# fateshelled/sycl_points

Measured on AMD Instinct MI355X. Metric: gicp_correspondences_per_sec, higher is better.
Workload: dtype f32

## Files before the change

sycl_points_amd/_lib.py:

```python
import ctypes as C
import os
import subprocess

_HERE = os.path.dirname(os.path.abspath(__file__))
LIB_PATH = os.environ.get("SP_AMD_LIB") or os.path.join(_HERE, "lib", "libsycl_points_amd.so")
CSRC = os.path.join(_HERE, "csrc")

SP_OK, SP_ERR_INVALID_ARGUMENT, SP_ERR_RUNTIME, SP_ERR_HIP = 0, 1, 2, 3
COMM_ID_BYTES = 128


class SpError(RuntimeError):

    def __init__(self, code, msg):
        super().__init__(f"[sycl_points_amd] error {code}: {msg}")
        self.code = code


class Linearized(C.Structure):
    _fields_ = [("H", C.c_float * 36), ("b", C.c_float * 6), ("error", C.c_float), ("inlier", C.c_uint32),
                ("inlier_lo", C.c_float), ("inlier_hi", C.c_float), ("pad", C.c_float * 2)]


class FactorParams(C.Structure):
# ... 344 lines not shown
    "sp_vhm_downsampling": (_i, [_vp, _vp, _f, _vp, _vp, _vp, _vp, _vp, _sz, C.POINTER(_sz), _vp]),
    "sp_vhm_overlap_ratio": (_i, [_vp, _vp, _sz, _vp, C.POINTER(_f), _vp]),
    "sp_vhm_remove_old_data": (_i, [_vp, _vp]),
    "sp_ogm_create": (_i, [_f, _vp, C.POINTER(_vp)]),
    "sp_ogm_destroy": (None, [_vp]),
    "sp_ogm_set": (_i, [_vp, _i, _f]),
    "sp_ogm_set_log_odds_limits": (_i, [_vp, _f, _f]),
    "sp_ogm_get": (_f, [_vp, _i]),
    "sp_ogm_info": (_sz, [_vp, _i]),
    "sp_ogm_clear": (_i, [_vp, _vp]),
    "sp_ogm_add_point_cloud": (_i, [_vp, _vp, _vp, _vp, _vp, _sz, _vp, _vp]),
    "sp_ogm_extract_occupied_points": (_i, [_vp, _vp, _f, _vp, _vp, _vp, _vp, _vp, _sz, C.POINTER(_sz), _vp]),
    "sp_ogm_extract_visible_points": (_i, [_vp, _vp, _f, _f, _f, _vp, _vp, _vp, _vp, _vp, _sz, C.POINTER(_sz), _vp]),
    "sp_ogm_overlap_ratio": (_i, [_vp, _vp, _sz, _vp, C.POINTER(_f), _vp]),
    "sp_ogm_voxel_probability": (_i, [_vp, _vp, C.POINTER(_f), _vp]),
    "sp_ogm_export": (_i, [_vp, _vp, _vp, _vp, _vp, _vp, _vp, _vp, _vp, _vp, _sz, C.POINTER(_sz), _vp]),
    "sp_pc2_resolve_fields_host": (_i, [C.POINTER(C.c_char_p), C.POINTER(C.c_uint32), C.POINTER(C.c_uint8), _sz, C.c_uint32, _i, _i, _i,
                                        C.POINTER(Pc2Layout)]),
    "sp_pc2_unpack_workspace_bytes": (_sz, [_sz]),
    "sp_pc2_unpack": (_i, [_vp, _sz, _sz, C.POINTER(Pc2Layout), _vp, _vp, _vp, _vp, _vp, _vp, _vp]),
    "sp_pc2_pack_point_step": (C.c_uint32, [_i, _i, _i]),
    "sp_pc2_pack": (_i, [_vp, _vp, _vp, _vp, _sz, C.c_double, _vp, _vp]),
    "sp_enhanced_reflectivity_workspace_bytes": (_sz, [_sz]),
    "sp_enhanced_reflectivity": (_i, [_vp, _vp, _sz, _vp, C.c_uint32, C.c_int32, _i, C.c_int32, _vp, _f, _f, _vp, _vp]),
}


INTERNAL_SIGNATURES = {
    "sp_internal_source_option": (_i, [_vp, _i, _i]),
    "sp_internal_grid_option": (_i, [_vp, _i, _i]),
    "sp_internal_bvh_option": (_i, [_vp, _i, _i]),
    "sp_internal_grid_small_build": (_i, [_i]),
    "sp_internal_align_searched_log": (_vp, [_vp, _vp]),
    "sp_internal_radix_sort_workspace_bytes": (_sz, [_sz]),
    "sp_internal_radix_sort_u32": (_i, [_vp, _vp, _vp, _vp, _sz, C.c_uint, _vp, _sz, _vp, _vp]),
    "sp_internal_radix_sort_u32_ex": (_i, [_vp, _vp, _vp, _vp, _sz, C.c_uint, C.c_uint, _i, _vp, _sz, _vp, _vp]),
    "sp_internal_radix_first_pass": (None, [_sz, C.c_uint, _vp]),
    "sp_internal_radix_sort_u64": (_i, [_vp, _vp, _vp, _vp, _sz, C.c_uint, _vp, _sz, _vp, _vp]),
    "sp_internal_exclusive_scan_workspace_bytes": (_sz, [_sz]),
    "sp_internal_exclusive_scan_u32": (_i, [_vp, _vp, _sz, _vp, _vp, _sz, _vp]),
    "sp_internal_atan2f_host": (None, [_vp, _vp, _sz, _vp]),
    "sp_internal_fps": (_i, [_i, _vp, _sz, _sz, C.c_uint32, _vp, _vp, _vp, _vp, _sz, _vp]),
    "sp_internal_eigen3": (_i, [_vp, _sz, _vp, _vp, _vp]),
    "sp_internal_inverse3": (_i, [_vp, _sz, _vp, _vp]),
}
VOXEL_BOX_SHARDS, VOXEL_BOX_SHARD_STRIDE = 16, 32
COORD = {"LIDAR": 0, "CAMERA": 1}
FPS_FORM = {"auto": 0, "one_workgroup": 1, "per_sample": 2, "persistent": 3}
INTERNAL_OPTION = {"stage_mask": 0, "reuse": 1, "fast_nn": 2, "self_knn_mode": 3, "persistent": 4, "persistent_from": 5,
                   "bvh_self_heap": 6, "bvh_sort_queries": 7, "grid_sort_queries": 8, "opt_wave_query": 9, "opt_fuse_trials": 10}


def build(force=False):
    srcs = [os.path.join(CSRC, f) for f in os.listdir(CSRC) if f.endswith((".hip", ".h"))]
    srcs.append(os.path.join(_HERE, "..", "include", "sycl_points_amd.h"))
    stale = (not os.path.exists(LIB_PATH)) or any(os.path.getmtime(s) > os.path.getmtime(LIB_PATH) for s in srcs)
    if force or stale:
        subprocess.check_call(["make", "-C", CSRC, "-j8", "-s"])
    return LIB_PATH


_lib = None


def lib():
    global _lib
# ... 21 lines not shown
```

sycl_points_amd/csrc/registration.hip:

```cpp
#include <algorithm>
#include <mutex>

#include "registration_device.h"
#include "sp_cov_normal.h"

namespace sp {
namespace {


struct PointTerm {
    float H[6][6];
    float b[6];
    float sq;
    float residual_norm;
    float genz_weight;
};

__device__ __forceinline__ void se3_jacobian(const Rigid& T, float px, float py, float pz, float J[3][6]) {
#pragma unroll
    for (int i = 0; i < 3; ++i) {
        const float r0 = T.R[i][0], r1 = T.R[i][1], r2 = T.R[i][2];
        J[i][0] = chain3(r0, 0.0f, r1, pz, r2, -py);
        J[i][1] = chain3(r0, -pz, r1, 0.0f, r2, px);
        J[i][2] = chain3(r0, py, r1, -px, r2, 0.0f);
// ... 374 lines not shown
    constexpr float kShrink = 0.25f * (1.0f - 1e-3f);
    rho2[o] = fminf(d23[3 * (size_t)i + 1], bound2) * kShrink;
    const int u1 = idx3[3 * (size_t)i + 1];
    float4 r = make_float4(INFINITY, INFINITY, INFINITY, 0.0f);
    if (u1 >= 0) {
        const float4 p = gpts[inv[u1]];
        r.x = p.x; r.y = p.y; r.z = p.z;
    }
    r.w = fminf(d23[3 * (size_t)i + 2], bound2) * kShrink;
    nb[i] = r;
}

__global__ __launch_bounds__(kBlock) void query_cell_kernel(const float4* __restrict__ pts, unsigned n, GridDesc g,
                                                            Mat4Arg T_val, const float* __restrict__ T_dev,
                                                            unsigned* __restrict__ keys, unsigned* __restrict__ vals) {
    const unsigned i = blockIdx.x * kBlock + threadIdx.x;
    if (i >= n) return;
    const Rigid T = load_rigid_colmajor(T_dev ? T_dev : T_val.m);
    const float4 p = pts[i];
    float qx, qy, qz;
    transform_point(T, p.x, p.y, p.z, qx, qy, qz);
    unsigned key = (unsigned)g.nx * g.ny * g.nz;
    if (isfinite(qx) && isfinite(qy) && isfinite(qz)) {
        const int cx = cell_coord(qx, g.ox, g.inv_h, g.nx), cy = cell_coord(qy, g.oy, g.inv_h, g.ny),
                  cz = cell_coord(qz, g.oz, g.inv_h, g.nz);
        key = ((unsigned)cz * g.ny + cy) * g.nx + cx;
    }
    keys[i] = key;
    vals[i] = i;
}
__global__ __launch_bounds__(kBlock) void prepare_source_kernel(const float4* __restrict__ pts,
                                                                const float4* __restrict__ covs,
                                                                unsigned* __restrict__ order, bool identity, unsigned n,
                                                                unsigned stride, float* __restrict__ out_pts,
                                                                float* __restrict__ out_covp) {
    const unsigned i = blockIdx.x * kBlock + threadIdx.x;
    if (i >= n) return;
    const unsigned src = identity ? i : order[i];
    if (identity) order[i] = i;
    const float4 p = pts[src];
    out_pts[i] = p.x; out_pts[stride + i] = p.y; out_pts[2 * (size_t)stride + i] = p.z;
    if (!covs) return;
    const Mat3 P = plane_regularize(load_cov(covs + 4 * (size_t)src));
    out_covp[i] = P.m[0][0];
    out_covp[stride + i] = (P.m[0][1] + P.m[1][0]) * 0.5f;
    out_covp[2 * (size_t)stride + i] = (P.m[0][2] + P.m[2][0]) * 0.5f;
    out_covp[3 * (size_t)stride + i] = P.m[1][1];
    out_covp[4 * (size_t)stride + i] = (P.m[1][2] + P.m[2][1]) * 0.5f;
    out_covp[5 * (size_t)stride + i] = P.m[2][2];
}


template <int LOSS, bool FAST_NN, bool P2D = false>
__global__ __launch_bounds__(kBlock) void gicp_fused_kernel(FusedParams P, float* __restrict__ partials) {
    const Rigid T = load_rigid_colmajor(P.T_dev ? P.T_dev : P.T_val.m);
    float acc[kAcc - 1];
#pragma unroll
    for (int e = 0; e < kAcc - 1; ++e) acc[e] = 0.0f;
    unsigned cnt = 0, searched = 0;
    for (unsigned i = blockIdx.x * kBlock + threadIdx.x; i < P.n; i += gridDim.x * kBlock)
        fused_point<LOSS, FAST_NN, P2D, kSeedSearches, kNegCert>(P, T, i, acc, cnt, searched);
    block_reduce_store<kAcc - 1>(acc, cnt, partials + (size_t)blockIdx.x * kPartial, false, searched);
}

template <int LOSS, bool P2D>
__global__ __launch_bounds__(kBlock) void error_prepared_kernel(FusedParams P, Mat4Arg T_lin_val, const float* T_lin_dev,
                                                                float* __restrict__ partials) {
    const Rigid T = load_rigid_colmajor(P.T_dev ? P.T_dev : P.T_val.m);
    const Rigid TL = load_rigid_colmajor(T_lin_dev ? T_lin_dev : T_lin_val.m);
    float acc[1] = {0.0f};
    unsigned cnt = 0;
    for (unsigned i = blockIdx.x * kBlock + threadIdx.x; i < P.n; i += gridDim.x * kBlock)
        error_prepared_point<LOSS, P2D>(P, T, TL, i, acc, cnt);
    block_reduce_store<1>(acc, cnt, partials + (size_t)blockIdx.x * kPartial);
}


struct AlignState {
    float T[16];
    float T_lin[16];
    float delta[8];
    unsigned converged;
// ... 689 lines not shown
    }
    if (certificates) {
        const int rc2 = build_certificates(t, as_stream(stream));
        if (rc2 != SP_OK) { sp_gicp_target_destroy(t); return rc2; }
    }
    const int rc = sp_gicp_target_update(t, tgt_covs, stream);
    if (rc != SP_OK) { sp_gicp_target_destroy(t); return rc; }
    *out = t;
    return SP_OK;
}
}
}

extern "C" int sp_gicp_target_create(const sp_grid* grid, const float* tgt_covs, size_t n, void* stream,
                                     sp_gicp_target** out) {
    return sp::target_create(grid, tgt_covs, n, true, stream, out);
}
extern "C" int sp_gicp_target_create_plain(const sp_grid* grid, const float* tgt_covs, size_t n, void* stream,
                                           sp_gicp_target** out) {
    return sp::target_create(grid, tgt_covs, n, false, stream, out);
}
extern "C" int sp_gicp_target_certify(sp_gicp_target* t, const float* tgt_covs, void* stream) {
    if (!t || !tgt_covs) return SP_ERR_INVALID_ARGUMENT;
    if (t->rho2 != nullptr) return SP_OK;
    t->note(sp::as_stream(stream));
    const int rc = sp::build_certificates(t, sp::as_stream(stream));
    if (rc != SP_OK) return rc;
    return sp_gicp_target_update(t, tgt_covs, stream);
}
extern "C" int sp_gicp_target_has_certificates(const sp_gicp_target* t) { return t && t->rho2 != nullptr ? 1 : 0; }

extern "C" void sp_gicp_source_destroy(sp_gicp_source* s) {
    if (!s) return;
    (void)hipFree(s->pts); (void)hipFree(s->covp); (void)hipFree(s->perm); (void)hipFree(s->ccache); (void)hipFree(s->ccache2); (void)hipFree(s->qcert); (void)hipFree(s->qcert2); (void)hipFree(s->opt_rows);
    (void)hipFree(s->keys_in); (void)hipFree(s->keys_out); (void)hipFree(s->vals_in); (void)hipFree(s->sort_tmp);
    delete s;
}
extern "C" int sp_gicp_source_create(size_t n_max, sp_gicp_source** out) {
    using namespace sp;
    if (!out) return SP_ERR_INVALID_ARGUMENT;
    *out = nullptr;
    if (n_max >= (1ull << 32)) { sp_set_error("[Registration] more than 2^32 source points"); return SP_ERR_INVALID_ARGUMENT; }
    sp_gicp_source* s = new sp_gicp_source();
    s->n_max = n_max;
    const size_t n = n_max ? n_max : 1;
    s->sort_tmp_bytes = radix_sort_u32_workspace_bytes(n);
    hipError_t e = hipMalloc(&s->pts, (n + 64) * sizeof(float4));
    if (e == hipSuccess) e = hipMalloc(&s->covp, (n + 64) * 2 * sizeof(float4));
    if (e == hipSuccess) e = hipMalloc(&s->perm, n * 4);
    if (e == hipSuccess) e = hipMalloc(&s->ccache, n * 3 * sizeof(float4));
    if (e == hipSuccess) e = hipMalloc(&s->ccache2, std::min<size_t>(n, 2048) * 3 * sizeof(float4));
    s->qcert_points = std::min<size_t>(n, 131072);
    if (e == hipSuccess) e = hipMalloc(&s->qcert, s->qcert_points * sizeof(float4));
    if (e == hipSuccess) e = hipMalloc(&s->qcert2, std::min<size_t>(n, 2048) * sizeof(float4));
    if (e == hipSuccess) e = hipMalloc(&s->opt_rows, sp::kOptRowsBytes);
    if (e == hipSuccess) e = hipMemset(s->opt_rows, 0, sp::kOptRowsBytes);
    if (e == hipSuccess) e = hipMalloc(&s->keys_in, n * 4);
    if (e == hipSuccess) e = hipMalloc(&s->keys_out, n * 4);
    if (e == hipSuccess) e = hipMalloc(&s->vals_in, n * 4);
    if (e == hipSuccess) e = hipMalloc(&s->sort_tmp, s->sort_tmp_bytes ? s->sort_tmp_bytes : 16);
    if (e != hipSuccess) {
        sp_set_error(hipGetErrorString(e));
        sp_gicp_source_destroy(s);
        return SP_ERR_HIP;
    }
    *out = s;
    return SP_OK;
}
extern "C" int sp_gicp_source_prepare(sp_gicp_source* s, const sp_gicp_target* target, const float* src_points,
                                      const float* src_covs, size_t n, const float* transT, int transT_on_device,
                                      int sort_by_cell, void* stream) {
    using namespace sp;
    if (!s || !target) return SP_ERR_INVALID_ARGUMENT;
    if (n > s->n_max) {
        sp_set_error("[sp_gicp_source_prepare] more points than the object was created for");
        return SP_ERR_INVALID_ARGUMENT;
    }
    if (!src_covs && n && target->reg_type == SP_REG_GICP) {
        sp_set_error("[Registration::validate_params] Covariance matrices of source and target must be pre-computed "
                     "before performing GICP matching.");
        return SP_ERR_RUNTIME;
    }
    s->n = n;
    s->sorted = sort_by_cell != 0;
    if (n == 0) return SP_OK;
    hipStream_t st = as_stream(stream);
    const float4* pts = reinterpret_cast<const float4*>(src_points);
    const unsigned nb = div_up(n, kBlock);
    if (sort_by_cell == SP_SOURCE_SORT) {
        Mat4Arg tv;
        for (int i = 0; i < 16; ++i) tv.m[i] = (i % 5 == 0) ? 1.0f : 0.0f;
        if (transT && !transT_on_device)
            for (int i = 0; i < 16; ++i) tv.m[i] = transT[i];
        const GridDesc g = grid_desc(target->grid);
        query_cell_kernel<<<nb, kBlock, 0, st>>>(pts, (unsigned)n, g, tv, transT_on_device ? transT : nullptr, s->keys_in,
                                                 s->vals_in);
        unsigned end_bit = 1;
        while ((1ull << end_bit) <= target->grid->ncells && end_bit < 32) ++end_bit;
        const unsigned begin_bit = end_bit > 16 ? end_bit - 16 : 0;
        bool in_b = false;
        if (radix_sort_pairs_u32(s->keys_in, s->keys_out, s->vals_in, s->perm, n, end_bit, s->sort_tmp, s->sort_tmp_bytes, &in_b,
                                 st, begin_bit) != SP_OK) {
            sp_set_error("[Registration] radix sort of the source failed");
            return SP_ERR_HIP;
        }
        if (!in_b) { unsigned* t = s->perm; s->perm = s->vals_in; s->vals_in = t; }
    }
    s->cache_valid = false;
    s->qcert_valid = false;
    s->cache_target = target;
    s->cache_version = target->version;
    prepare_source_kernel<<<nb, kBlock, 0, st>>>(pts, target->reg_type == SP_REG_GICP ? reinterpret_cast<const float4*>(src_covs) : nullptr,
                                                 s->perm, sort_by_cell != SP_SOURCE_SORT, (unsigned)n,
                                                 (unsigned)((n + 63) / 64 * 64), reinterpret_cast<float*>(s->pts),
                                                 reinterpret_cast<float*>(s->covp));
    return launch_status();
}



extern "C" int sp_gicp_iteration_fused(const sp_gicp_target* target, const sp_gicp_source* source, float* transT,
                                       int transT_on_device, const sp_factor_params* params, const sp_gn_params* gn,
                                       int32_t* nn_idx_out, float* nn_d2_out, sp_linearized* out, float* delta_out8,
                                       void* workspace, size_t workspace_bytes, void* stream) {
    using namespace sp;
    hipStream_t st = as_stream(stream);
    if (!target || !source || !params || !out) return SP_ERR_INVALID_ARGUMENT;
    if (const int rc = check_prepared_reg(target, params); rc != SP_OK) return rc;
    if (gn && !transT_on_device) {
        sp_set_error("[sp_gicp_iteration_fused] the fused Gauss-Newton update needs the pose on the device");
        return SP_ERR_INVALID_ARGUMENT;
    }
    const size_t n = source->n;
    if (n == 0) return zero_async(out, sizeof(sp_linearized), st);
    if (const int rc = check_workspace(workspace, workspace_bytes, n); rc != SP_OK) return rc;
    target->note(st);
    const FusedParams P = make_fused_params(target, source, params, transT, transT_on_device, nn_idx_out, nn_d2_out);
    const bool fills_cache = P.ccache != nullptr && (source->opt_stage_mask & 1);
    const unsigned grid = reduce_grid(n);
    float* partials = static_cast<float*>(workspace);
    const int rc = with_variant(params->robust_type, source_fast_nn(source), params->reg_type == SP_REG_POINT_TO_DISTRIBUTION,
                                [&](auto L, auto FAST_NN, auto P2D) {
        if (source->opt_stage_mask & 1)
            gicp_fused_kernel<L, FAST_NN, P2D><<<grid, kBlock, 0, st>>>(P, partials);
        return SP_OK;
    });
    if (rc != SP_OK) return rc;
    if (fills_cache) { source->cache_valid = true; source->qcert_valid = false; }
// ... 327 lines not shown
        for (int k = 0; k < k_tail; ++k) {
            const int rc = sp_gicp_align_step(target, source, transT_device, params, gn, k, 0, nn_idx_out, nn_d2_out, lin_out,
                                              workspace, workspace_bytes, stream);
            if (rc != SP_OK) { persist_release(guard, st); return rc; }
        }
        return launch_persistent(target, source, transT_device, params, gn, k_tail, max_iterations, nn_idx_out, nn_d2_out, lin_out,
                                 delta_out8, iterations_out, workspace, st, guard);
    }
    for (int k = 0; k < max_iterations; ++k) {
        const int rc = sp_gicp_align_step(target, source, transT_device, params, gn, k, 0, nn_idx_out, nn_d2_out, lin_out,
                                          workspace, workspace_bytes, stream);
        if (rc != SP_OK) return rc;
    }
    return sp_gicp_align_finish(source, transT_device, gn, max_iterations - 1, 0, lin_out, delta_out8, iterations_out,
                                workspace, workspace_bytes, stream);
}

extern "C" int sp_gicp_source_set_persistent(sp_gicp_source* s, int enable) {
    if (!s) return SP_ERR_INVALID_ARGUMENT;
    s->opt_persistent = enable ? 1 : 0;
    return SP_OK;
}

extern "C" int sp_gicp_source_set_wave_per_point(sp_gicp_source* s, int mode) {
    if (!s || mode < 0 || mode > 2) return SP_ERR_INVALID_ARGUMENT;
    s->opt_wave_query = mode;
    return SP_OK;
}

extern "C" const uint32_t* sp_internal_align_searched_log(void* workspace, size_t* n_entries_out) {
    if (n_entries_out) *n_entries_out = sp::kSearchedLog;
    return workspace ? sp::align_ws(workspace).searched_log : nullptr;
}
extern "C" int sp_internal_source_option(sp_gicp_source* s, int option, int value) {
    if (!s) return SP_ERR_INVALID_ARGUMENT;
    switch (option) {
        case SP_INTERNAL_FUSED_STAGE_MASK: s->opt_stage_mask = value; return SP_OK;
        case SP_INTERNAL_FUSED_REUSE: s->opt_reuse = value; s->cache_valid = false; return SP_OK;
        case SP_INTERNAL_FUSED_FAST_NN: s->opt_fast_nn = value; return SP_OK;
        case SP_INTERNAL_FUSED_PERSISTENT: s->opt_persistent = value; return SP_OK;
        case SP_INTERNAL_FUSED_PERSISTENT_FROM: s->opt_persistent_from = value < 0 ? 0 : value; return SP_OK;
        case SP_INTERNAL_OPT_WAVE_QUERY: s->opt_wave_query = value; return SP_OK;
        case SP_INTERNAL_OPT_FUSE_TRIALS: s->opt_fuse_trials = value; return SP_OK;
    }
    return SP_ERR_INVALID_ARGUMENT;
}
```

sycl_points_amd/csrc/registration_device.h:

```cpp
#ifndef SP_REGISTRATION_DEVICE_H
#define SP_REGISTRATION_DEVICE_H

#include "grid_device.h"
#include "radix_sort.h"
#include "sp_xchg.h"

#include <type_traits>

void sp_set_error(const char* msg);

#include "sp_internal.h"

namespace sp {
namespace {

constexpr int kAcc = 29;
constexpr int kPartial = 32;
constexpr int kMaxBlocks = 1024;

template <bool SC1>
__device__ __forceinline__ void store_row_word(float* p, float v) {
    if (SC1) __hip_atomic_store(p, v, __ATOMIC_RELAXED, __HIP_MEMORY_SCOPE_AGENT);
    else *p = v;
}
// ... 155 lines not shown
                                               float crit_trans, float* delta_out8, bool fold_inlier, LdltScratch& w) {
    if (fold_inlier) lin->inlier = (uint32_t)lin->inlier_hi * 4096u + (uint32_t)lin->inlier_lo;
    float H[36], nb[6], delta[6];
#pragma unroll
    for (int i = 0; i < 36; ++i) H[i] = lin->H[i];
#pragma unroll
    for (int i = 0; i < 6; ++i) {
        H[i * 6 + i] = lin->H[i * 6 + i] + lambda * 1.0f;
        nb[i] = -lin->b[i];
    }
    const bool ok = ldlt6_solve(H, nb, delta, w);
    const float nr = sqrtf(delta[0] * delta[0] + delta[1] * delta[1] + delta[2] * delta[2]);
    const float nt = sqrtf(delta[3] * delta[3] + delta[4] * delta[4] + delta[5] * delta[5]);
    const bool conv = ok && (nr < crit_rot) && (nt < crit_trans);
    const Rigid cur = load_rigid_colmajor(T);
    const Rigid upd = rigid_mul(cur, se3_exp(delta));
    store_rigid_colmajor(upd, T);
    if (delta_out8) {
        for (int i = 0; i < 6; ++i) delta_out8[i] = delta[i];
        delta_out8[6] = conv ? 1.0f : 0.0f;
        delta_out8[7] = ok ? 1.0f : 0.0f;
    }
}

struct Sym3 {
    float xx, xy, xz, yy, yz, zz;
};

__device__ __forceinline__ Sym3 load_sym(const float4* __restrict__ p) {
    const float4 a = p[0], b = p[1];
    return Sym3{a.x, a.y, a.z, a.w, b.x, b.y};
}

struct FusedParams {
    const float* src;
    const float* scovp;
    unsigned sstride;
    const float4* tpts;
    const unsigned* tstart;
    const float4* tcovp;
    const float4* tnb;
    GridDesc g;
    unsigned n;
    float max_d2, scale;
    Mat4Arg T_val;
    const float* T_dev;
    const unsigned* perm;
    float4* ccache;
    int cache_valid;
    int32_t* nn_idx;
    float* nn_d2;
};

template <int LOSS, bool P2D = false, bool ERR_ONLY = false, int NACC = kAcc - 1>
__device__ __forceinline__ void fused_math(const FusedParams& P, const Rigid& T, const float4 s, float qx, float qy,
                                           float qz, const Nearest& nn, const Sym3& Cs, const Sym3& Ct,
                                           float (&acc)[NACC], unsigned& cnt) {
    const float r0 = nn.x - qx, r1 = nn.y - qy, r2 = nn.z - qz;
    const float (&R)[3][3] = T.R;
    float W[3][3];
#pragma unroll
    for (int j = 0; j < 3; ++j) {
        W[0][j] = chain3(Ct.xx, R[0][j], Ct.xy, R[1][j], Ct.xz, R[2][j]);
        W[1][j] = chain3(Ct.xy, R[0][j], Ct.yy, R[1][j], Ct.yz, R[2][j]);
        W[2][j] = chain3(Ct.xz, R[0][j], Ct.yz, R[1][j], Ct.zz, R[2][j]);
    }
    const float g00 = chain3(R[0][0], W[0][0], R[1][0], W[1][0], R[2][0], W[2][0]);
    const float g01 = chain3(R[0][0], W[0][1], R[1][0], W[1][1], R[2][0], W[2][1]);
    const float g02 = chain3(R[0][0], W[0][2], R[1][0], W[1][2], R[2][0], W[2][2]);
    const float g11 = chain3(R[0][1], W[0][1], R[1][1], W[1][1], R[2][1], W[2][1]);
    const float g12 = chain3(R[0][1], W[0][2], R[1][1], W[1][2], R[2][1], W[2][2]);
    const float g22 = chain3(R[0][2], W[0][2], R[1][2], W[1][2], R[2][2], W[2][2]);
    float n00, n01, n02, n11, n12, n22;
    if constexpr (P2D) {
        n00 = g00; n01 = g01; n02 = g02; n11 = g11; n12 = g12; n22 = g22;
    } else {
        const float a00 = g00 + Cs.xx, a01 = g01 + Cs.xy, a02 = g02 + Cs.xz, a11 = g11 + Cs.yy, a12 = g12 + Cs.yz,
                    a22 = g22 + Cs.zz;
        const float c00 = fmaf(a11, a22, -a12 * a12);
        const float c01 = fmaf(a02, a12, -a01 * a22);
        const float c02 = fmaf(a01, a12, -a02 * a11);
        const float det = fmaf(a00, c00, fmaf(a01, c01, a02 * c02));
        const float inv_det = fabsf(det) < 1e-6f ? 0.0f : 1.0f / det;
        n00 = c00 * inv_det; n01 = c01 * inv_det; n02 = c02 * inv_det;
        n11 = fmaf(a00, a22, -a02 * a02) * inv_det;
// ... 41 lines not shown
        r1 = c0;
        r2 = make_float4(c1.x, c1.y, __int_as_float(nn.idx), __uint_as_float(nn.pos));
        Ct = Sym3{c0.x, c0.y, c0.z, c0.w, c1.x, c1.y};
    }
    row[0] = r0;
    row[1] = r1;
    row[2] = r2;
}

__device__ __forceinline__ bool certified(const FusedParams& P, float d, float rho2, float qx, float qy, float qz,
                                          unsigned pos) {
    if (d < rho2) return true;
    if (!P.tnb || !(rho2 > 0.0f)) return false;
    const float4 nb = P.tnb[pos];
    return d < nb.w && d < dist2(qx, qy, qz, nb.x, nb.y, nb.z);
}

__device__ __forceinline__ float search_bound2(const FusedParams& P) {
    return (P.nn_idx == nullptr && P.max_d2 < FLT_MAX) ? __uint_as_float(__float_as_uint(P.max_d2) + 1u) : FLT_MAX;
}
__device__ __forceinline__ float search_bound2_margin(const FusedParams& P, float& margin2) {
    margin2 = 0.0f;
    if (P.nn_idx != nullptr || !(P.max_d2 < FLT_MAX) || P.ccache == nullptr) return search_bound2(P);
    const float B = sqrtf(P.max_d2), m = 0.25f * B;
    const float wide = (B + m) * (B + m);
    if (!(wide < FLT_MAX)) return search_bound2(P);
    margin2 = (0.98f * m) * (0.98f * m);
    return wide;
}

template <int LOSS, bool FAST_NN, bool P2D = false, bool SEED = true, bool NEG = true>
__device__ __forceinline__ void fused_point(const FusedParams& P, const Rigid& T, unsigned i, float (&acc)[kAcc - 1],
                                            unsigned& cnt, unsigned& searched) {
    const float4 s = make_float4(P.src[i], P.src[P.sstride + i], P.src[2 * (size_t)P.sstride + i], 1.0f);
    float qx, qy, qz;
    transform_point(T, s.x, s.y, s.z, qx, qy, qz);
    Nearest nn;
    Sym3 Ct{0.0f, 0.0f, 0.0f, 0.0f, 0.0f, 0.0f};
    bool hit = false;
    bool seeded = false;
    Nearest seed;
    seed.d2 = FLT_MAX; seed.idx = -1; seed.pos = 0; seed.x = seed.y = seed.z = 0.0f;
    float4* const row = P.ccache ? P.ccache + 3 * (size_t)i : nullptr;
    if (row && P.cache_valid) {
        const float4 r0 = row[0], r1 = row[1], r2 = row[2];
        const float d = dist2(qx, qy, qz, r0.x, r0.y, r0.z);
        const unsigned pos = __float_as_uint(r2.w);
        if (certified(P, d, r0.w, qx, qy, qz, pos)) {
            hit = true;
            nn.idx = __float_as_int(r2.z); nn.pos = pos; nn.x = r0.x; nn.y = r0.y; nn.z = r0.z;
            nn.d2 = nn.idx >= 0 ? d : FLT_MAX;
            Ct = Sym3{r1.x, r1.y, r1.z, r1.w, r2.x, r2.y};
        } else if (SEED && __float_as_int(r2.z) >= 0) {
            seed.d2 = d; seed.idx = __float_as_int(r2.z); seed.pos = pos; seed.x = r0.x; seed.y = r0.y; seed.z = r0.z;
            seeded = true;
        }
    }
    if (!hit) {
        ++searched;
        float margin2 = 0.0f;
        const float bound2 = NEG ? search_bound2_margin(P, margin2) : search_bound2(P);
        seeded = seeded && seed.d2 < bound2;
        if (!seeded) { seed.d2 = bound2; seed.idx = -1; seed.pos = 0; seed.x = seed.y = seed.z = 0.0f; }
        if (FAST_NN) {
            nn = grid_nn1_auto(P.tpts, P.tstart, P.g, qx, qy, qz, bound2, &seed);
        } else {
            nn = grid_nn1(P.tpts, P.tstart, P.g, qx, qy, qz, &seed, 0);
        }
        if (row) {
            if (NEG) store_correspondence(row, P, nn, Ct, qx, qy, qz, margin2);
            else store_correspondence(row, P, nn, Ct);
        } else if (nn.idx >= 0) Ct = load_sym(P.tcovp + 2 * (size_t)nn.pos);
    }
    if (P.nn_idx) {
        const unsigned o = P.perm[i];
        P.nn_idx[o] = nn.idx;
        P.nn_d2[o] = nn.d2;
    }
    if (nn.idx < 0 || nn.d2 > P.max_d2) return;
    const float* const cp = P.scovp + i;
    const size_t st = P.sstride;
    const Sym3 Cs = P2D ? Sym3{0.0f, 0.0f, 0.0f, 0.0f, 0.0f, 0.0f}
                        : Sym3{cp[0], cp[st], cp[2 * st], cp[3 * st], cp[4 * st], cp[5 * st]};
    fused_math<LOSS, P2D>(P, T, s, qx, qy, qz, nn, Cs, Ct, acc, cnt);
}

#ifdef SP_OPT_TIMING
__device__ unsigned long long g_sp_dbg[24 * 16];
__device__ unsigned g_sp_step;
__device__ unsigned long long g_sp_wg[24 * 8];
#define SP_PSTAMP(k) if (blockIdx.x == 0 && threadIdx.x == 0 && g_sp_step < 24) g_sp_dbg[g_sp_step * 16 + (k)] = wall_clock64()
#else
#define SP_PSTAMP(k)
#endif
template <int LOSS, bool P2D = false>
__device__ __forceinline__ void fused_point_wave(const FusedParams& P, const Rigid& T, unsigned i, bool valid,
                                                 float (&acc)[kAcc - 1], unsigned& cnt, unsigned& searched) {
    const unsigned ii = valid ? i : 0u;
    SP_PSTAMP(0);
    const float4 s = make_float4(P.src[ii], P.src[P.sstride + ii], P.src[2 * (size_t)P.sstride + ii], 1.0f);
    float qx, qy, qz;
    transform_point(T, s.x, s.y, s.z, qx, qy, qz);
    Nearest nn;
    nn.d2 = FLT_MAX; nn.idx = -1; nn.pos = 0; nn.x = nn.y = nn.z = 0.0f;
    Sym3 Ct{0.0f, 0.0f, 0.0f, 0.0f, 0.0f, 0.0f};
    bool hit = false;
    float4* const row = P.ccache + 3 * (size_t)ii;
    Nearest seed;
    seed.d2 = FLT_MAX; seed.idx = -1; seed.pos = 0; seed.x = seed.y = seed.z = 0.0f;
    if (valid && P.cache_valid) {
        const float4 r0 = row[0], r1 = row[1], r2 = row[2];
        const float d = dist2(qx, qy, qz, r0.x, r0.y, r0.z);
        const unsigned pos = __float_as_uint(r2.w);
        if (certified(P, d, r0.w, qx, qy, qz, pos)) {
            hit = true;
            nn.idx = __float_as_int(r2.z); nn.pos = pos; nn.x = r0.x; nn.y = r0.y; nn.z = r0.z;
            nn.d2 = nn.idx >= 0 ? d : FLT_MAX;
            Ct = Sym3{r1.x, r1.y, r1.z, r1.w, r2.x, r2.y};
        } else if (__float_as_int(r2.z) >= 0) {
            seed.d2 = d; seed.idx = __float_as_int(r2.z); seed.pos = pos; seed.x = r0.x; seed.y = r0.y; seed.z = r0.z;
        }
    }
    const bool search = valid && !hit;
    SP_PSTAMP(1);
    float margin2 = 0.0f;
    const float bound2 = search_bound2_margin(P, margin2);
    bool open = false;
    bool fast_ok = true;
    const bool seeded = search && seed.d2 < bound2;
    if (search) {
        ++searched;
        if (!seeded) { seed.d2 = bound2; seed.idx = -1; seed.pos = 0; seed.x = seed.y = seed.z = 0.0f; }
        fast_ok = grid_nn1_fast(P.tpts, P.tstart, P.g, qx, qy, qz, nn, bound2, &seed);
    }
    SP_PSTAMP(2);
    if (search && !fast_ok) open = !grid_nn1_block4(P.tpts, P.tstart, P.g, qx, qy, qz, nn);
    SP_PSTAMP(3);
#ifdef SP_OPT_TIMING
    if (blockIdx.x == 0 && threadIdx.x < 64) {
        const unsigned long long a = __ballot(search), b = __ballot(search && !fast_ok), c = __ballot(open);
        const unsigned long long sd = __ballot(seeded);
        if (threadIdx.x == 0 && g_sp_step < 24) {
            unsigned long long* const d = g_sp_dbg + g_sp_step * 16;
            d[8] = __popcll(a); d[9] = __popcll(b); d[10] = __popcll(c); d[11] = __popcll(sd);
        }
    }
#endif
    if (__ballot(open)) {
        if (open && !(nn.d2 < FLT_MAX)) {
            const Nearest seed = nn;
            nn = grid_nn1(P.tpts, P.tstart, P.g, qx, qy, qz, &seed, 2);
            open = false;
        }
        grid_nn1_ball_wave(P.tpts, P.tstart, P.g, open, qx, qy, qz, nn);
    }
    SP_PSTAMP(4);
    if (search) store_correspondence(row, P, nn, Ct, qx, qy, qz, margin2);
    SP_PSTAMP(5);
    if (valid && P.nn_idx) {
        const unsigned o = P.perm[ii];
        P.nn_idx[o] = nn.idx;
        P.nn_d2[o] = nn.d2;
    }
    if (!valid || nn.idx < 0 || nn.d2 > P.max_d2) return;
    const float* const cp = P.scovp + ii;
    const size_t st = P.sstride;
    const Sym3 Cs = P2D ? Sym3{0.0f, 0.0f, 0.0f, 0.0f, 0.0f, 0.0f}
                        : Sym3{cp[0], cp[st], cp[2 * st], cp[3 * st], cp[4 * st], cp[5 * st]};
    fused_math<LOSS, P2D>(P, T, s, qx, qy, qz, nn, Cs, Ct, acc, cnt);
    SP_PSTAMP(6);
}

template <int LOSS, bool P2D = false>
__device__ __forceinline__ void fused_query_wave(const FusedParams& P, const Rigid& T, unsigned i, float (&acc)[kAcc - 1],
                                                 unsigned& cnt, unsigned& searched, float4* rows_out = nullptr,
                                                 const float4* qc_in = nullptr, float4* qc_out = nullptr) {
    SP_PSTAMP(0);
    const float4 s = make_float4(P.src[i], P.src[P.sstride + i], P.src[2 * (size_t)P.sstride + i], 1.0f);
    float qx, qy, qz;
    transform_point(T, s.x, s.y, s.z, qx, qy, qz);
    Nearest nn;
    nn.d2 = FLT_MAX; nn.idx = -1; nn.pos = 0; nn.x = nn.y = nn.z = 0.0f;
    Sym3 Ct{0.0f, 0.0f, 0.0f, 0.0f, 0.0f, 0.0f};
    bool hit = false, seeded = false;
    float moved2 = 0.0f;
    float4* const row = P.ccache + 3 * (size_t)i;
    float4* const row_out = rows_out ? rows_out + 3 * (size_t)i : row;
    if (qc_in != nullptr && qc_out == nullptr) qc_out = const_cast<float4*>(qc_in);
    if (P.cache_valid) {
        const float4 r0 = row[0], r1 = row[1], r2 = row[2];
        const float4 qc = qc_in ? qc_in[i] : make_float4(0.0f, 0.0f, 0.0f, 0.0f);
        const float d = dist2(qx, qy, qz, r0.x, r0.y, r0.z);
        const unsigned pos = __float_as_uint(r2.w);
        const bool real = __float_as_int(r2.z) >= 0;
        if (qc_in) moved2 = dist2(qx, qy, qz, qc.x, qc.y, qc.z);
        if (certified(P, d, r0.w, qx, qy, qz, pos) || (qc_in && real && moved2 < qc.w)) {
            hit = true;
            nn.idx = __float_as_int(r2.z); nn.pos = pos; nn.x = r0.x; nn.y = r0.y; nn.z = r0.z;
            nn.d2 = nn.idx >= 0 ? d : FLT_MAX;
            Ct = Sym3{r1.x, r1.y, r1.z, r1.w, r2.x, r2.y};
            if (row_out != row) { row_out[0] = r0; row_out[1] = r1; row_out[2] = r2; }
            if (qc_out && qc_out != qc_in) qc_out[i] = qc;
        } else if (real) {
            nn.d2 = d; nn.idx = __float_as_int(r2.z); nn.pos = pos; nn.x = r0.x; nn.y = r0.y; nn.z = r0.z;
            seeded = true;
        }
    }
    SP_PSTAMP(1);
    if (!hit) {
        ++searched;
        float margin2 = 0.0f;
        const float bound2 = search_bound2_margin(P, margin2);
        float second2 = 0.0f, d1 = 0.0f;
        if (seeded && nn.d2 < bound2) {
            const float pad = qc_in ? fminf(2.0f * sqrtf(moved2), 0.25f * P.g.h) : 0.0f;
            const float reach = sqrtf(nn.d2) + pad;
            grid_nn1_query_wave(P.tpts, P.tstart, P.g, qx, qy, qz, fminf(reach * reach, bound2), nn, second2);
        } else {
            const float half = 0.5f * P.g.h;
            const float first2 = fminf(half * half, bound2);
            nn.d2 = first2; nn.idx = -1; nn.pos = 0; nn.x = nn.y = nn.z = 0.0f;
            grid_nn1_query_wave(P.tpts, P.tstart, P.g, qx, qy, qz, first2, nn, second2);
            if (nn.idx < 0 && first2 < bound2) {
                nn.d2 = bound2;
                grid_nn1_query_wave(P.tpts, P.tstart, P.g, qx, qy, qz, bound2, nn, second2);
            }
        }
        d1 = nn.d2;
        if (nn.idx < 0) nn.d2 = FLT_MAX;
        SP_PSTAMP(2); SP_PSTAMP(3); SP_PSTAMP(4);
        store_correspondence(row_out, P, nn, Ct, qx, qy, qz, margin2);
        if (qc_out) {
            float m = 0.0f;
            if (nn.idx >= 0) {
                const float scale = fmaxf(fmaxf(fabsf(qx), fabsf(qy)), fmaxf(fabsf(qz), 1.0f));
                m = 0.475f * (sqrtf(second2) - sqrtf(d1)) - 2.0e-6f * scale;
                m = fminf(fmaxf(m, 0.0f), P.g.h);
            }
            qc_out[i] = make_float4(qx, qy, qz, m * m);
        }
        SP_PSTAMP(5);
    }
    if (nn.idx < 0 || nn.d2 > P.max_d2) return;
    const float* const cp = P.scovp + i;
    const size_t st = P.sstride;
    const Sym3 Cs = P2D ? Sym3{0.0f, 0.0f, 0.0f, 0.0f, 0.0f, 0.0f}
                        : Sym3{cp[0], cp[st], cp[2 * st], cp[3 * st], cp[4 * st], cp[5 * st]};
    fused_math<LOSS, P2D>(P, T, s, qx, qy, qz, nn, Cs, Ct, acc, cnt);
    SP_PSTAMP(6);
}

template <int LOSS, bool P2D>
__device__ __forceinline__ void error_prepared_point(const FusedParams& P, const Rigid& T, const Rigid& TL, unsigned i,
                                                     float (&acc)[1], unsigned& cnt) {
    const float4 s = make_float4(P.src[i], P.src[P.sstride + i], P.src[2 * (size_t)P.sstride + i], 1.0f);
    const float4* const row = P.ccache + 3 * (size_t)i;
    const float4 tp = row[0], c0 = row[1], c1 = row[2];
    if (__float_as_int(c1.z) < 0) return;
    float lx, ly, lz;
    transform_point(TL, s.x, s.y, s.z, lx, ly, lz);
    if (dist2(lx, ly, lz, tp.x, tp.y, tp.z) > P.max_d2) return;
    float qx, qy, qz;
    transform_point(T, s.x, s.y, s.z, qx, qy, qz);
    Nearest nn;
    nn.x = tp.x; nn.y = tp.y; nn.z = tp.z; nn.idx = __float_as_int(c1.z); nn.pos = 0; nn.d2 = 0.0f;
    const float* const cp = P.scovp + i;
    const size_t st = P.sstride;
    Sym3 Cs{0.0f, 0.0f, 0.0f, 0.0f, 0.0f, 0.0f};
    if (!P2D) Cs = Sym3{cp[0], cp[st], cp[2 * st], cp[3 * st], cp[4 * st], cp[5 * st]};
    const Sym3 Ct{c0.x, c0.y, c0.z, c0.w, c1.x, c1.y};
    fused_math<LOSS, P2D, true, 1>(P, T, s, qx, qy, qz, nn, Cs, Ct, acc, cnt);
}

template <int NV, int BLOCK>
__device__ __forceinline__ void block_reduce_lds(float (&acc)[NV], unsigned cnt, unsigned extra, float* __restrict__ tot) {
    __shared__ float red[BLOCK / kWave][kPartial];
    const unsigned lane = threadIdx.x & (kWave - 1), wave = threadIdx.x / kWave;
#pragma unroll
    for (int e = 0; e < NV; ++e) acc[e] = wave_sum_to_lane63(acc[e]);
    cnt = wave_sum_u32_to_lane63(cnt);
    extra = wave_sum_u32_to_lane63(extra);
    if (lane == kWave - 1) {
#pragma unroll
        for (int e = 0; e < NV; ++e) red[wave][e] = acc[e];
        red[wave][NV] = __uint_as_float(cnt);
        red[wave][NV + 1] = __uint_as_float(extra);
    }
    __syncthreads();
    if (threadIdx.x < NV) {
        float s = 0.0f;
#pragma unroll
        for (int w = 0; w < BLOCK / kWave; ++w) s += red[w][threadIdx.x];
        tot[threadIdx.x] = s;
    } else if (threadIdx.x == NV || threadIdx.x == NV + 1) {
        unsigned c = 0;
#pragma unroll
        for (int w = 0; w < BLOCK / kWave; ++w) c += __float_as_uint(red[w][threadIdx.x]);
        tot[threadIdx.x] = threadIdx.x == NV ? __uint_as_float(c) : (float)c;
    }
    __syncthreads();
}

// ... 38 lines not shown
}
__device__ __forceinline__ bool grid_wait(unsigned* tickets, unsigned want, unsigned long long budget) {
    const unsigned long long t0 = wall_clock64();
    for (;;) {
        unsigned have = 0;
#pragma unroll
        for (int sh = 0; sh < kTicketShards; ++sh)
            have += __hip_atomic_load(tickets + sh * kTicketStride, __ATOMIC_RELAXED, __HIP_MEMORY_SCOPE_AGENT);
        if (have >= want) return true;
        if (wall_clock64() - t0 > budget) return false;
        __builtin_amdgcn_s_sleep(2);
    }
}

}
}

struct sp_gicp_target {
    const sp_grid* grid = nullptr;
    float4* covp = nullptr;
    float* rho2 = nullptr;
    float4* nb = nullptr;
    unsigned long long version = 0;
    int reg_type = SP_REG_GICP;
    size_t n = 0;
    mutable sp::StreamSet streams;
    void note(hipStream_t st) const { streams.note(st); if (grid) sp::grid_use(grid, st); }
};
namespace sp {
constexpr size_t kOptRowsBytes = 2 * (size_t)256 * 32 * sizeof(unsigned long long);
}
struct sp_gicp_source {
    size_t n_max = 0, n = 0;
    float4* pts = nullptr;
    float4* covp = nullptr;
    unsigned* perm = nullptr;
    float4* ccache = nullptr;
    float4* qcert = nullptr;
    float4* qcert2 = nullptr;
    size_t qcert_points = 0;
    mutable bool qcert_valid = false;
    float4* ccache2 = nullptr;
    unsigned long long* opt_rows = nullptr;
    mutable unsigned opt_epoch = 0;
    mutable bool cache_valid = false;
    const sp_gicp_target* cache_target = nullptr;
    unsigned long long cache_version = 0;
    bool sorted = false;
    int opt_stage_mask = 3;
    int opt_reuse = 2;
    int opt_fast_nn = -1;
    int opt_persistent = 1;
    int opt_persistent_from = 4;
    int opt_fuse_trials = 1;
    int opt_wave_query = 1;
    unsigned *keys_in = nullptr, *keys_out = nullptr, *vals_in = nullptr;
    void* sort_tmp = nullptr;
    size_t sort_tmp_bytes = 0;
};

namespace sp {
namespace {
FusedParams make_fused_params(const sp_gicp_target* target, const sp_gicp_source* source, const sp_factor_params* params,
                              const float* transT, int transT_on_device, int32_t* nn_idx_out, float* nn_d2_out) {
    const size_t n = source->n;
    FusedParams P;
    P.src = reinterpret_cast<const float*>(source->pts);
    P.scovp = reinterpret_cast<const float*>(source->covp);
    P.sstride = (unsigned)((n + 63) / 64 * 64);
    P.tpts = target->grid->d_pts;
    P.tstart = target->grid->d_start;
    P.tcovp = target->covp;
    P.tnb = source->opt_reuse > 1 ? target->nb : nullptr;
    P.g = grid_desc(target->grid);
    P.n = (unsigned)n;
    P.max_d2 = params->max_correspondence_distance * params->max_correspondence_distance;
    P.scale = params->robust_scale;
    for (int i = 0; i < 16; ++i) P.T_val.m[i] = (i % 5 == 0) ? 1.0f : 0.0f;
    if (transT && !transT_on_device)
        for (int i = 0; i < 16; ++i) P.T_val.m[i] = transT[i];
    P.T_dev = transT_on_device ? transT : nullptr;
    P.perm = source->perm;
    P.ccache = source->ccache;
    P.cache_valid = (source->opt_reuse && source->cache_valid && source->cache_target == target &&
                     source->cache_version == target->version) ? 1 : 0;
    P.nn_idx = (nn_idx_out && nn_d2_out) ? nn_idx_out : nullptr;
    P.nn_d2 = nn_d2_out;
    return P;
}

int check_prepared_reg(const sp_gicp_target* target, const sp_factor_params* params) {
    if (params->reg_type != SP_REG_GICP && params->reg_type != SP_REG_POINT_TO_DISTRIBUTION) {
        sp_set_error("[sp_gicp_*] only RegType::GICP and RegType::POINT_TO_DISTRIBUTION have a prepared/fused form");
        return SP_ERR_INVALID_ARGUMENT;
    }
    if (params->reg_type != target->reg_type) {
        sp_set_error("[sp_gicp_*] the prepared target holds the rows of another RegType: call sp_gicp_target_prepare");
        return SP_ERR_INVALID_ARGUMENT;
    }
    if (params->rotation_constraint_enable) {
        sp_set_error("[sp_gicp_*] the rotation constraint needs the raw covariances: use sp_gicp_linearize");
        return SP_ERR_INVALID_ARGUMENT;
// ... 83 lines not shown
```

sycl_points_amd/csrc/sp_internal.h:

```cpp
#ifndef SP_INTERNAL_H
#define SP_INTERNAL_H

#include "../../include/sycl_points_amd.h"

#ifdef __cplusplus
extern "C" {
#endif

enum {
    SP_INTERNAL_FUSED_STAGE_MASK = 0,
    SP_INTERNAL_FUSED_REUSE = 1,
    SP_INTERNAL_FUSED_FAST_NN = 2,
    SP_INTERNAL_SELF_KNN_MODE = 3,
    SP_INTERNAL_FUSED_PERSISTENT = 4,
    SP_INTERNAL_FUSED_PERSISTENT_FROM = 5,
    SP_INTERNAL_BVH_SELF_HEAP = 6,
    SP_INTERNAL_BVH_SORT_QUERIES = 7,
    SP_INTERNAL_GRID_SORT_QUERIES = 8,
    SP_INTERNAL_OPT_WAVE_QUERY = 9,
    SP_INTERNAL_OPT_FUSE_TRIALS = 10
};

int sp_internal_source_option(sp_gicp_source* source, int option, int value);
int sp_internal_grid_option(sp_grid* grid, int option, int value);
int sp_internal_bvh_option(sp_bvh* bvh, int option, int value);
int sp_internal_grid_small_build(int enable);
const uint32_t* sp_internal_align_searched_log(void* workspace, size_t* n_entries_out);
size_t sp_internal_radix_sort_workspace_bytes(size_t n);
int sp_internal_radix_sort_u32(uint32_t* keys_a, uint32_t* keys_b, uint32_t* vals_a, uint32_t* vals_b, size_t n,
                               unsigned bits, void* workspace, size_t workspace_bytes, int* result_in_b_out, void* stream);
int sp_internal_radix_sort_u32_ex(uint32_t* keys_a, uint32_t* keys_b, uint32_t* vals_a, uint32_t* vals_b, size_t n,
                                  unsigned bits, unsigned first_bit, int first_hist_ready, void* workspace,
                                  size_t workspace_bytes, int* result_in_b_out, void* stream);
void sp_internal_radix_first_pass(size_t n, unsigned bits, unsigned* out4);
int sp_internal_radix_sort_u64(uint64_t* keys_a, uint64_t* keys_b, uint32_t* vals_a, uint32_t* vals_b, size_t n,
                               unsigned bits, void* workspace, size_t workspace_bytes, int* result_in_b_out, void* stream);
size_t sp_internal_exclusive_scan_workspace_bytes(size_t n);
int sp_internal_exclusive_scan_u32(const uint32_t* in, uint32_t* out, size_t n, uint32_t* total_out_or_null, void* workspace,
                                   size_t workspace_bytes, void* stream);
void sp_internal_atan2f_host(const float* y, const float* x, size_t n, float* out);
int sp_internal_fps(int form, const float* points, size_t n, size_t sampling_num, uint32_t first_index, uint32_t* order_out,
                    uint8_t* flags_out_opt, float* min_d2_out_opt, void* workspace, size_t workspace_bytes, void* stream);
int sp_internal_eigen3(const float* covs, size_t n, float* vals_out, float* vecs_out, void* stream);
int sp_internal_inverse3(const float* mats, size_t n, float* out, void* stream);

#ifdef __cplusplus
}
#endif
#endif
```

Baseline: 30.03 billion.

## Interleave source points and covariances into per-wave tiled planes

Replaces the separate strided SoA arrays for source points and plane-regularized covariances with one buffer of per-wave tiles of 9 planes, so each wave's point and covariance words sit contiguously. This is meant to improve locality and cut address arithmetic when the fused GICP kernels load source data. It also removes the null check on the correspondence cache row in fused_point and recomputes the tile address behind an asm barrier to limit register pressure. Internal copy helpers for the tile buffer are added. The loss of the ccache null check assumes the cache is always allocated.

```diff
diff --git a/sycl_points_amd/_lib.py b/sycl_points_amd/_lib.py
--- a/sycl_points_amd/_lib.py
+++ b/sycl_points_amd/_lib.py
@@ -400,6 +400,8 @@
     "sp_internal_bvh_option": (_i, [_vp, _i, _i]),
     "sp_internal_grid_small_build": (_i, [_i]),
     "sp_internal_align_searched_log": (_vp, [_vp, _vp]),
+    "sp_internal_source_tile_floats": (_sz, [_vp]),
+    "sp_internal_source_tiles_copy": (_i, [_vp, _vp, _sz, _i, _vp]),
     "sp_internal_radix_sort_workspace_bytes": (_sz, [_sz]),
     "sp_internal_radix_sort_u32": (_i, [_vp, _vp, _vp, _vp, _sz, C.c_uint, _vp, _sz, _vp, _vp]),
     "sp_internal_radix_sort_u32_ex": (_i, [_vp, _vp, _vp, _vp, _sz, C.c_uint, C.c_uint, _i, _vp, _sz, _vp, _vp]),
diff --git a/sycl_points_amd/csrc/registration.hip b/sycl_points_amd/csrc/registration.hip
--- a/sycl_points_amd/csrc/registration.hip
+++ b/sycl_points_amd/csrc/registration.hip
@@ -430,22 +430,22 @@
 __global__ __launch_bounds__(kBlock) void prepare_source_kernel(const float4* __restrict__ pts,
                                                                 const float4* __restrict__ covs,
                                                                 unsigned* __restrict__ order, bool identity, unsigned n,
-                                                                unsigned stride, float* __restrict__ out_pts,
-                                                                float* __restrict__ out_covp) {
+                                                                float* __restrict__ tiles) {
     const unsigned i = blockIdx.x * kBlock + threadIdx.x;
     if (i >= n) return;
     const unsigned src = identity ? i : order[i];
     if (identity) order[i] = i;
     const float4 p = pts[src];
-    out_pts[i] = p.x; out_pts[stride + i] = p.y; out_pts[2 * (size_t)stride + i] = p.z;
+    float* const w = tiles + ((size_t)(i / kWave) * kSrcTileWords + (i % kWave));
+    w[0] = p.x; w[kWave] = p.y; w[2 * kWave] = p.z;
     if (!covs) return;
     const Mat3 P = plane_regularize(load_cov(covs + 4 * (size_t)src));
-    out_covp[i] = P.m[0][0];
-    out_covp[stride + i] = (P.m[0][1] + P.m[1][0]) * 0.5f;
-    out_covp[2 * (size_t)stride + i] = (P.m[0][2] + P.m[2][0]) * 0.5f;
-    out_covp[3 * (size_t)stride + i] = P.m[1][1];
-    out_covp[4 * (size_t)stride + i] = (P.m[1][2] + P.m[2][1]) * 0.5f;
-    out_covp[5 * (size_t)stride + i] = P.m[2][2];
+    w[3 * kWave] = P.m[0][0];
+    w[4 * kWave] = (P.m[0][1] + P.m[1][0]) * 0.5f;
+    w[5 * kWave] = (P.m[0][2] + P.m[2][0]) * 0.5f;
+    w[6 * kWave] = P.m[1][1];
+    w[7 * kWave] = (P.m[1][2] + P.m[2][1]) * 0.5f;
+    w[8 * kWave] = P.m[2][2];
 }
 
 
@@ -1201,7 +1201,7 @@
 
 extern "C" void sp_gicp_source_destroy(sp_gicp_source* s) {
     if (!s) return;
-    (void)hipFree(s->pts); (void)hipFree(s->covp); (void)hipFree(s->perm); (void)hipFree(s->ccache); (void)hipFree(s->ccache2); (void)hipFree(s->qcert); (void)hipFree(s->qcert2); (void)hipFree(s->opt_rows);
+    (void)hipFree(s->tiles); (void)hipFree(s->perm); (void)hipFree(s->ccache); (void)hipFree(s->ccache2); (void)hipFree(s->qcert); (void)hipFree(s->qcert2); (void)hipFree(s->opt_rows);
     (void)hipFree(s->keys_in); (void)hipFree(s->keys_out); (void)hipFree(s->vals_in); (void)hipFree(s->sort_tmp);
     delete s;
 }
@@ -1214,8 +1214,7 @@
     s->n_max = n_max;
     const size_t n = n_max ? n_max : 1;
     s->sort_tmp_bytes = radix_sort_u32_workspace_bytes(n);
-    hipError_t e = hipMalloc(&s->pts, (n + 64) * sizeof(float4));
-    if (e == hipSuccess) e = hipMalloc(&s->covp, (n + 64) * 2 * sizeof(float4));
+    hipError_t e = hipMalloc(&s->tiles, src_tile_words(n) * sizeof(float));
     if (e == hipSuccess) e = hipMalloc(&s->perm, n * 4);
     if (e == hipSuccess) e = hipMalloc(&s->ccache, n * 3 * sizeof(float4));
     if (e == hipSuccess) e = hipMalloc(&s->ccache2, std::min<size_t>(n, 2048) * 3 * sizeof(float4));
@@ -1280,9 +1279,7 @@
     s->cache_target = target;
     s->cache_version = target->version;
     prepare_source_kernel<<<nb, kBlock, 0, st>>>(pts, target->reg_type == SP_REG_GICP ? reinterpret_cast<const float4*>(src_covs) : nullptr,
-                                                 s->perm, sort_by_cell != SP_SOURCE_SORT, (unsigned)n,
-                                                 (unsigned)((n + 63) / 64 * 64), reinterpret_cast<float*>(s->pts),
-                                                 reinterpret_cast<float*>(s->covp));
+                                                 s->perm, sort_by_cell != SP_SOURCE_SORT, (unsigned)n, s->tiles);
     return launch_status();
 }
 
@@ -1676,6 +1673,16 @@
     if (n_entries_out) *n_entries_out = sp::kSearchedLog;
     return workspace ? sp::align_ws(workspace).searched_log : nullptr;
 }
+extern "C" size_t sp_internal_source_tile_floats(const sp_gicp_source* s) {
+    return s ? sp::src_tile_words(s->n_max ? s->n_max : 1) : 0;
+}
+extern "C" int sp_internal_source_tiles_copy(sp_gicp_source* s, float* device_buffer, size_t n_floats, int to_source, void* stream) {
+    if (!s || !device_buffer || n_floats != sp_internal_source_tile_floats(s)) return SP_ERR_INVALID_ARGUMENT;
+    const hipError_t e = hipMemcpyAsync(to_source ? s->tiles : device_buffer, to_source ? device_buffer : s->tiles,
+                                        n_floats * sizeof(float), hipMemcpyDeviceToDevice, sp::as_stream(stream));
+    if (e != hipSuccess) { sp_set_error(hipGetErrorString(e)); return SP_ERR_HIP; }
+    return SP_OK;
+}
 extern "C" int sp_internal_source_option(sp_gicp_source* s, int option, int value) {
     if (!s) return SP_ERR_INVALID_ARGUMENT;
     switch (option) {
diff --git a/sycl_points_amd/csrc/registration_device.h b/sycl_points_amd/csrc/registration_device.h
--- a/sycl_points_amd/csrc/registration_device.h
+++ b/sycl_points_amd/csrc/registration_device.h
@@ -211,10 +211,12 @@
     return Sym3{a.x, a.y, a.z, a.w, b.x, b.y};
 }
 
+constexpr unsigned kSrcPlanes = 9;
+constexpr unsigned kSrcTileWords = kSrcPlanes * kWave;
+__host__ __device__ inline size_t src_tile_words(size_t n) { return (n + kWave - 1) / kWave * kSrcTileWords; }
+
 struct FusedParams {
     const float* src;
-    const float* scovp;
-    unsigned sstride;
     const float4* tpts;
     const unsigned* tstart;
     const float4* tcovp;
@@ -230,6 +232,16 @@
     int32_t* nn_idx;
     float* nn_d2;
 };
+
+__device__ __forceinline__ const float* src_words(const FusedParams& P, unsigned i) {
+    return P.src + ((size_t)(i / kWave) * kSrcTileWords + (i % kWave));
+}
+__device__ __forceinline__ float4 src_point(const float* __restrict__ w) {
+    return make_float4(w[0], w[kWave], w[2 * kWave], 1.0f);
+}
+__device__ __forceinline__ Sym3 src_cov(const float* __restrict__ w) {
+    return Sym3{w[3 * kWave], w[4 * kWave], w[5 * kWave], w[6 * kWave], w[7 * kWave], w[8 * kWave]};
+}
 
 template <int LOSS, bool P2D = false, bool ERR_ONLY = false, int NACC = kAcc - 1>
 __device__ __forceinline__ void fused_math(const FusedParams& P, const Rigid& T, const float4 s, float qx, float qy,
@@ -337,7 +349,9 @@
 template <int LOSS, bool FAST_NN, bool P2D = false, bool SEED = true, bool NEG = true>
 __device__ __forceinline__ void fused_point(const FusedParams& P, const Rigid& T, unsigned i, float (&acc)[kAcc - 1],
                                             unsigned& cnt, unsigned& searched) {
-    const float4 s = make_float4(P.src[i], P.src[P.sstride + i], P.src[2 * (size_t)P.sstride + i], 1.0f);
+    const float* const sw = src_words(P, i);
+    const float4 s = src_point(sw);
+    float4* const row = P.ccache + 3 * (size_t)i;
     float qx, qy, qz;
     transform_point(T, s.x, s.y, s.z, qx, qy, qz);
     Nearest nn;
@@ -346,8 +360,7 @@
     bool seeded = false;
     Nearest seed;
     seed.d2 = FLT_MAX; seed.idx = -1; seed.pos = 0; seed.x = seed.y = seed.z = 0.0f;
-    float4* const row = P.ccache ? P.ccache + 3 * (size_t)i : nullptr;
-    if (row && P.cache_valid) {
+    if (P.cache_valid) {
         const float4 r0 = row[0], r1 = row[1], r2 = row[2];
         const float d = dist2(qx, qy, qz, r0.x, r0.y, r0.z);
         const unsigned pos = __float_as_uint(r2.w);
@@ -372,10 +385,8 @@
         } else {
             nn = grid_nn1(P.tpts, P.tstart, P.g, qx, qy, qz, &seed, 0);
         }
-        if (row) {
-            if (NEG) store_correspondence(row, P, nn, Ct, qx, qy, qz, margin2);
-            else store_correspondence(row, P, nn, Ct);
-        } else if (nn.idx >= 0) Ct = load_sym(P.tcovp + 2 * (size_t)nn.pos);
+        if (NEG) store_correspondence(row, P, nn, Ct, qx, qy, qz, margin2);
+        else store_correspondence(row, P, nn, Ct);
     }
     if (P.nn_idx) {
         const unsigned o = P.perm[i];
@@ -383,11 +394,11 @@
         P.nn_d2[o] = nn.d2;
     }
     if (nn.idx < 0 || nn.d2 > P.max_d2) return;
-    const float* const cp = P.scovp + i;
-    const size_t st = P.sstride;
-    const Sym3 Cs = P2D ? Sym3{0.0f, 0.0f, 0.0f, 0.0f, 0.0f, 0.0f}
-                        : Sym3{cp[0], cp[st], cp[2 * st], cp[3 * st], cp[4 * st], cp[5 * st]};
-    fused_math<LOSS, P2D>(P, T, s, qx, qy, qz, nn, Cs, Ct, acc, cnt);
+    unsigned i_again = i;
+    asm volatile("" : "+v"(i_again));
+    const float* const sw_again = src_words(P, i_again);
+    const Sym3 Cs = P2D ? Sym3{0.0f, 0.0f, 0.0f, 0.0f, 0.0f, 0.0f} : src_cov(sw_again);
+    fused_math<LOSS, P2D>(P, T, src_point(sw_again), qx, qy, qz, nn, Cs, Ct, acc, cnt);
 }
 
 #ifdef SP_OPT_TIMING
@@ -403,7 +414,8 @@
                                                  float (&acc)[kAcc - 1], unsigned& cnt, unsigned& searched) {
     const unsigned ii = valid ? i : 0u;
     SP_PSTAMP(0);
-    const float4 s = make_float4(P.src[ii], P.src[P.sstride + ii], P.src[2 * (size_t)P.sstride + ii], 1.0f);
+    const float* const sw = src_words(P, ii);
+    const float4 s = src_point(sw);
     float qx, qy, qz;
     transform_point(T, s.x, s.y, s.z, qx, qy, qz);
     Nearest nn;
@@ -468,10 +480,7 @@
         P.nn_d2[o] = nn.d2;
     }
     if (!valid || nn.idx < 0 || nn.d2 > P.max_d2) return;
-    const float* const cp = P.scovp + ii;
-    const size_t st = P.sstride;
-    const Sym3 Cs = P2D ? Sym3{0.0f, 0.0f, 0.0f, 0.0f, 0.0f, 0.0f}
-                        : Sym3{cp[0], cp[st], cp[2 * st], cp[3 * st], cp[4 * st], cp[5 * st]};
+    const Sym3 Cs = P2D ? Sym3{0.0f, 0.0f, 0.0f, 0.0f, 0.0f, 0.0f} : src_cov(sw);
     fused_math<LOSS, P2D>(P, T, s, qx, qy, qz, nn, Cs, Ct, acc, cnt);
     SP_PSTAMP(6);
 }
@@ -481,7 +490,8 @@
                                                  unsigned& cnt, unsigned& searched, float4* rows_out = nullptr,
                                                  const float4* qc_in = nullptr, float4* qc_out = nullptr) {
     SP_PSTAMP(0);
-    const float4 s = make_float4(P.src[i], P.src[P.sstride + i], P.src[2 * (size_t)P.sstride + i], 1.0f);
+    const float* const sw = src_words(P, i);
+    const float4 s = src_point(sw);
     float qx, qy, qz;
     transform_point(T, s.x, s.y, s.z, qx, qy, qz);
     Nearest nn;
@@ -547,10 +557,7 @@
         SP_PSTAMP(5);
     }
     if (nn.idx < 0 || nn.d2 > P.max_d2) return;
-    const float* const cp = P.scovp + i;
-    const size_t st = P.sstride;
-    const Sym3 Cs = P2D ? Sym3{0.0f, 0.0f, 0.0f, 0.0f, 0.0f, 0.0f}
-                        : Sym3{cp[0], cp[st], cp[2 * st], cp[3 * st], cp[4 * st], cp[5 * st]};
+    const Sym3 Cs = P2D ? Sym3{0.0f, 0.0f, 0.0f, 0.0f, 0.0f, 0.0f} : src_cov(sw);
     fused_math<LOSS, P2D>(P, T, s, qx, qy, qz, nn, Cs, Ct, acc, cnt);
     SP_PSTAMP(6);
 }
@@ -558,7 +565,8 @@
 template <int LOSS, bool P2D>
 __device__ __forceinline__ void error_prepared_point(const FusedParams& P, const Rigid& T, const Rigid& TL, unsigned i,
                                                      float (&acc)[1], unsigned& cnt) {
-    const float4 s = make_float4(P.src[i], P.src[P.sstride + i], P.src[2 * (size_t)P.sstride + i], 1.0f);
+    const float* const sw = src_words(P, i);
+    const float4 s = src_point(sw);
     const float4* const row = P.ccache + 3 * (size_t)i;
     const float4 tp = row[0], c0 = row[1], c1 = row[2];
     if (__float_as_int(c1.z) < 0) return;
@@ -569,10 +577,8 @@
     transform_point(T, s.x, s.y, s.z, qx, qy, qz);
     Nearest nn;
     nn.x = tp.x; nn.y = tp.y; nn.z = tp.z; nn.idx = __float_as_int(c1.z); nn.pos = 0; nn.d2 = 0.0f;
-    const float* const cp = P.scovp + i;
-    const size_t st = P.sstride;
     Sym3 Cs{0.0f, 0.0f, 0.0f, 0.0f, 0.0f, 0.0f};
-    if (!P2D) Cs = Sym3{cp[0], cp[st], cp[2 * st], cp[3 * st], cp[4 * st], cp[5 * st]};
+    if (!P2D) Cs = src_cov(sw);
     const Sym3 Ct{c0.x, c0.y, c0.z, c0.w, c1.x, c1.y};
     fused_math<LOSS, P2D, true, 1>(P, T, s, qx, qy, qz, nn, Cs, Ct, acc, cnt);
 }
@@ -677,8 +683,7 @@
 }
 struct sp_gicp_source {
     size_t n_max = 0, n = 0;
-    float4* pts = nullptr;
-    float4* covp = nullptr;
+    float* tiles = nullptr;
     unsigned* perm = nullptr;
     float4* ccache = nullptr;
     float4* qcert = nullptr;
@@ -710,9 +715,7 @@
                               const float* transT, int transT_on_device, int32_t* nn_idx_out, float* nn_d2_out) {
     const size_t n = source->n;
     FusedParams P;
-    P.src = reinterpret_cast<const float*>(source->pts);
-    P.scovp = reinterpret_cast<const float*>(source->covp);
-    P.sstride = (unsigned)((n + 63) / 64 * 64);
+    P.src = source->tiles;
     P.tpts = target->grid->d_pts;
     P.tstart = target->grid->d_start;
     P.tcovp = target->covp;
diff --git a/sycl_points_amd/csrc/sp_internal.h b/sycl_points_amd/csrc/sp_internal.h
--- a/sycl_points_amd/csrc/sp_internal.h
+++ b/sycl_points_amd/csrc/sp_internal.h
@@ -26,6 +26,8 @@
 int sp_internal_bvh_option(sp_bvh* bvh, int option, int value);
 int sp_internal_grid_small_build(int enable);
 const uint32_t* sp_internal_align_searched_log(void* workspace, size_t* n_entries_out);
+size_t sp_internal_source_tile_floats(const sp_gicp_source* source);
+int sp_internal_source_tiles_copy(sp_gicp_source* source, float* device_buffer, size_t n_floats, int to_source, void* stream);
 size_t sp_internal_radix_sort_workspace_bytes(size_t n);
 int sp_internal_radix_sort_u32(uint32_t* keys_a, uint32_t* keys_b, uint32_t* vals_a, uint32_t* vals_b, size_t n,
                                unsigned bits, void* workspace, size_t workspace_bytes, int* result_in_b_out, void* stream);
```

Measured after the change: 30.70 billion (median of 6 runs). 2.2% higher.
